# igmsalinas/unet-rir

Measured on AMD Instinct MI355X. Metric: RIR spectrograms/sec (train step) on [B,2,256,256] U-Net, higher is better.
Workload: dtype bf16; 1 GPU; UNet 4 down/4 up, number_filters_0=64, kernels=3, per-GPU batch 32 of [2,256,256] + [2,16] (BASELINE.json configs[1] per GPU; global batch 32), full train step: fwd + loss + bwd + grad all-reduce + Adam; bf16 activations/gradients, fp32 accumulate/statistics/master weights; global_batch=32, parallelism=dp1, rccl_world_size=1, params=68613058, driven_by=Trainer.step(UNetEngine), schedule=side-stream weight gradients + bucket-wise Adam

## Files before the change

unet-rir_amd/build.py:

```python
import os
import subprocess
import sys
from concurrent.futures import ThreadPoolExecutor

HERE = os.path.dirname(os.path.abspath(__file__))
CSRC = os.path.join(HERE, "csrc")
OBJ = os.path.join(HERE, "build")
LIB = os.path.join(HERE, "libunetrir.so")
SOURCES = ["igemm.hip", "api.hip", "elementwise.hip", "head.hip", "head_mfma.hip", "head1x1.hip", "head_up2.hip", "wgrad3x3.hip", "wgrad3x3r.hip", "wgrad3x3g.hip", "wgrad3x3d.hip", "igemm_bf16.hip", "conv3x3.hip", "conv3x3r.hip", "conv3x3g.hip", "conv3x3h.hip", "conv3x3s.hip", "conv3x3d.hip", "conv3x3p.hip", "upconv3x3.hip", "upconv3x3g.hip", "upconv3x3q.hip", "features.hip", "dense.hip", "stem3x3.hip", "pw1x1.hip", "conv2x2.hip", "igemm2_bf16.hip", "weights.hip", "splitk_reduce.hip", "evalmetrics.hip", "acoustics.hip", "vae.hip", "vq.hip", "dataset.hip", "griffinlim.hip", "lamb.hip"]
FLAGS = ["-O3", "--offload-arch=gfx950", "-std=c++17", "-fPIC", "-Wno-unused-value"]


def _headers():
    return [os.path.join(CSRC, f) for f in os.listdir(CSRC) if f.endswith(".h")] + [
        os.path.join(os.path.dirname(HERE), "include", "unetrir.h")]


def _stale(target, deps):
    if not os.path.exists(target):
        return True
    t = os.path.getmtime(target)
    return any(os.path.getmtime(d) > t for d in deps)


def needs_build():
    deps = [os.path.join(CSRC, f) for f in os.listdir(CSRC)] + _headers()
    return _stale(LIB, deps)


def build(force=False, verbose=False, extra_flags=(), lib=LIB, obj_dir=OBJ):
    if not force and lib == LIB and not needs_build():
        return LIB
    hipcc = os.environ.get("HIPCC", "/opt/rocm/bin/hipcc")
    os.makedirs(obj_dir, exist_ok=True)
    hdrs = _headers()
    jobs = []
    for s in SOURCES:
        src = os.path.join(CSRC, s)
        obj = os.path.join(obj_dir, s[:-4] + ".o")
        if force or _stale(obj, [src] + hdrs):
            jobs.append([hipcc] + FLAGS + list(extra_flags) + ["-c", src, "-o", obj])

    def run(cmd):
        if verbose:
            print(" ".join(cmd), file=sys.stderr)
        subprocess.run(cmd, check=True)

    with ThreadPoolExecutor(max_workers=min(8, os.cpu_count() or 1)) as ex:
        list(ex.map(run, jobs))
    run([hipcc, "--offload-arch=gfx950", "-shared", "-fPIC", "-o", lib] +
        [os.path.join(obj_dir, s[:-4] + ".o") for s in SOURCES])
    return lib


ABL_LIB = os.path.join(HERE, "libunetrir_abl.so")


def build_ablations(verbose=False):
    return build(force=False, verbose=verbose, extra_flags=["-DUNETRIR_ABLATIONS"], lib=ABL_LIB, obj_dir=os.path.join(HERE, "build_abl"))


if __name__ == "__main__":
# ... 5 lines not shown
```

unet-rir_amd/csrc/api.hip:

```cpp
#include <hip/hip_runtime.h>
#include <cstdlib>
#include <cstring>
#include <atomic>
#include <mutex>
#include <utility>
#include <vector>
#include "kernels.h"

namespace {
int env_int(const char* name, int dflt) {
    const char* e = getenv(name);
    return e ? atoi(e) : dflt;
}
const unetrir_config* load_config() {
    unetrir_config* c = new unetrir_config;
    c->conv3x3 = env_int("UNETRIR_CONV3X3", 1);
    c->conv3x3g = env_int("UNETRIR_CONV3X3G", 1);
    c->conv3x3g_pair = env_int("UNETRIR_CONV3X3G_PAIR", 1);
    c->conv3x3h = env_int("UNETRIR_CONV3X3H", 1);
    c->conv3x3s = env_int("UNETRIR_CONV3X3S", 1);
    c->conv3x3r = env_int("UNETRIR_CONV3X3R", 1);
    c->stem = env_int("UNETRIR_STEM", 1);
    c->upconv3x3g = env_int("UNETRIR_UPCONV3X3G", 1);
    c->wgrad3x3g = env_int("UNETRIR_WGRAD3X3G", 1);
// ... 94 lines not shown
}

namespace {

struct Same { int out, before; };
inline Same same_geom(int n_in, int k, int s) {
    Same r;
    r.out = (n_in + s - 1) / s;
    int total = (r.out - 1) * s + k - n_in;
    if (total < 0) total = 0;
    r.before = total / 2;
    return r;
}

inline uint32_t pack_tap(int dy, int dx, int widx) {
    return (uint32_t)(uint8_t)(int8_t)dy | ((uint32_t)(uint8_t)(int8_t)dx << 8) | ((uint32_t)widx << 16);
}

inline bool geom_ok(const unetrir_conv_geom* g) {
    return g && g->B > 0 && g->H > 0 && g->W > 0 && g->Cin > 0 && g->Cout > 0 && g->k >= 1 && g->k <= 6 &&
           (g->stride == 1 || g->stride == 2);
}

struct ProfRec { int fam, tag; hipEvent_t e0, e1; double flops; };
std::mutex g_prof_mu;
bool g_prof_on = false;
unsigned g_prof_mask = ~0u;
std::vector<ProfRec> g_prof;

struct ProfScope {
    bool on; ProfRec r; hipStream_t s;
    ProfScope(int fam, double flops, hipStream_t st, int tag = -1) : on(g_prof_on && ((g_prof_mask >> fam) & 1u)), s(st) {
        if (!on) return;
        r.fam = fam; r.tag = tag; r.flops = flops;
        hipEventCreate(&r.e0); hipEventCreate(&r.e1);
        hipEventRecord(r.e0, s);
    }
    ~ProfScope() {
        if (!on) return;
        hipEventRecord(r.e1, s);
        std::lock_guard<std::mutex> lk(g_prof_mu);
        g_prof.push_back(r);
    }
};

inline double conv_flops(const unetrir_conv_geom* g) {
    const Same sy = same_geom(g->H, g->k, g->stride), sx = same_geom(g->W, g->k, g->stride);
    return 2.0 * g->B * sy.out * sx.out * (double)g->Cout * g->Cin * g->k * g->k;
}
inline int conv_family(const unetrir_conv_geom* g, int fam) {
    return (g->Cin <= 8 || g->Cout <= 8) ? 5 : fam;
}

enum class Kern { TAPTABLE, TAPTABLE_CLASSES, PATCH, STEM, CONV3X3G_PAIR, CONV3X3P, CONV3X3G, CONV3X3S, CONV3X3H, CONV3X3R, CONV3X3D,
                  UPCONV3X3, UPCONV3X3G, UPCONV3X3Q, PW1X1 };
struct ConvPlan {
    Kern kernel;
    long long colstat_rows;
};

enum Dir { FWD, DGRAD, TFWD };
struct ConvCall {
    const unetrir_conv_geom* g; Dir dir;
    const void* in; int ldi; const void* w; const void* wpk; const float* bias; const void* addend; int ldadd; void* out; int ldo;
    float* colstat;
};

inline double patch_util(int H, int W) { return (double)H * W / ((double)((H + 7) / 8 * 8) * ((W + 31) / 32 * 32)); }

Conv3Args conv3_args(const ConvCall& c) {
    const unetrir_conv_geom* g = c.g;
    const bool dg = c.dir != FWD;
    Conv3Args a{};
    a.in = c.in; a.ldi = c.ldi; a.w = c.w; a.bias = c.bias; a.addend = c.addend; a.ldadd = c.ldadd; a.out = c.out; a.ldo = c.ldo;
    a.colstat = c.colstat;
    a.B = g->B; a.H = g->H; a.W = g->W; a.C = dg ? g->Cout : g->Cin; a.N = dg ? g->Cin : g->Cout;
    if (g->stride == 1) {
        a.flip = dg ? 1 : UNETRIR_ABL(UNETRIR_ABL_HOST(), 256) ? 2 : 0;
    } else if (dg) {
        a.H = same_geom(g->H, 3, 2).out; a.W = same_geom(g->W, 3, 2).out;
    } else {
        a.wpk = (g->Cin % 64 == 0 && g->Cout % 64 == 0) ? c.wpk : nullptr;
    }
    return a;
}

PwArgs pw_args(const ConvCall& c) {
    const unetrir_conv_geom* g = c.g;
    const Same sy = same_geom(g->H, 1, g->stride), sx = same_geom(g->W, 1, g->stride);
    PwArgs a{};
    a.in = (const __bf16*)c.in; a.ldi = c.ldi; a.w = (const __bf16*)c.w; a.bias = c.bias; a.addend = (const __bf16*)c.addend;
    a.ldadd = c.ldadd; a.out = (__bf16*)c.out; a.ldo = c.ldo; a.colstat = c.colstat;
    a.B = g->B; a.PH = sy.out; a.PW = sx.out;
    if (c.dir == FWD) {
        a.IH = g->H; a.IW = g->W; a.OH = sy.out; a.OW = sx.out; a.SI = g->stride; a.SO = 1; a.C = g->Cin; a.N = g->Cout;
    } else {
        a.IH = sy.out; a.IW = sx.out; a.OH = g->H; a.OW = g->W; a.SI = 1; a.SO = g->stride; a.fill = g->stride == 2; a.C = g->Cout;
        a.N = g->Cin;
    }
    return a;
}

long long taptable_rows(const unetrir_conv_geom* g, Dir dir) {
    const Same sy = same_geom(g->H, g->k, g->stride), sx = same_geom(g->W, g->k, g->stride);
    if (dir == FWD) return igemm_colstat_rows((long long)g->B * sy.out * sx.out, g->Cout);
    if (g->stride == 1) return igemm_colstat_rows((long long)g->B * g->H * g->W, g->Cin);
    return 4 * igemm_colstat_rows((long long)g->B * sy.out * sx.out, g->Cin, 4);
}

ConvPlan plan_conv(const ConvCall& c, bool bf16, bool stats) {
    const unetrir_config& cfg = unetrir_cfg();
    const unetrir_conv_geom* g = c.g;
    if (g->k == 3 && g->stride == 1) {
        const Conv3Args a = conv3_args(c);
        const bool pair = bf16 && cfg.conv3x3g_pair && conv3x3g_pair_applies(a, cfg.conv3x3g_pair == 2);
        if ((cfg.conv3x3 && patch_util(g->H, g->W) >= 0.7) || pair) {
            if (!bf16) return {Kern::PATCH, 0};
            if (cfg.stem && !stats && stem3x3_applies(a)) return {Kern::STEM, 0};
            if (cfg.conv3x3g) {
                if (pair) return {Kern::CONV3X3G_PAIR, conv3x3g_colstat_rows(a, true)};
                if (cfg.conv3x3p && conv3x3p_applies(a)) return {Kern::CONV3X3P, conv3x3p_colstat_rows(a)};
                if (conv3x3g_applies(a)) return {Kern::CONV3X3G, conv3x3g_colstat_rows(a, false)};
            }
            if (cfg.conv3x3s && conv3x3s_applies(a)) return {Kern::CONV3X3S, conv3x3s_colstat_rows(a)};
            if (cfg.conv3x3h && conv3x3h_applies(a)) return {Kern::CONV3X3H, conv3x3h_colstat_rows(a)};
            if (cfg.conv3x3r && !(a.flip & 2)) return {Kern::CONV3X3R, conv3x3r_colstat_rows(a)};
            return {Kern::PATCH, 0};
        }
    }
    if (bf16 && g->k == 1 && cfg.pw1x1 && !(stats && c.addend) && pw1x1_applies(pw_args(c)))
        return {Kern::PW1X1, pw1x1_colstat_rows(pw_args(c))};
    if (g->stride == 1) return {Kern::TAPTABLE, taptable_rows(g, c.dir)};
    if (c.dir == FWD) {
        if (bf16 && g->k == 3 && cfg.conv3x3d && conv3x3d_applies(conv3_args(c))) return {Kern::CONV3X3D, 0};
        return {Kern::TAPTABLE, g->k == 3 ? 0 : taptable_rows(g, c.dir)};
    }
    const Same sy = same_geom(g->H, g->k, 2), sx = same_geom(g->W, g->k, 2);
    if (g->k == 3 && sy.before == 0 && sx.before == 0 && g->H == 2 * sy.out && g->W == 2 * sx.out && patch_util(sy.out, sx.out) >= 0.7) {
        const Conv3Args a = conv3_args(c);
        if (bf16 && cfg.upconv3x3g && upconv3x3g_applies(a))
            return {cfg.upconv3x3q && upconv3x3q_applies(a) ? Kern::UPCONV3X3Q : Kern::UPCONV3X3G, 0};
        if (cfg.conv3x3) return {Kern::UPCONV3X3, 0};
    }
    return {Kern::TAPTABLE_CLASSES, c.dir == TFWD && g->k != 3 ? taptable_rows(g, c.dir) : 0};
}

struct F32 {
    static constexpr int is_bf16 = 0;
    using T = float; using Args = IgemmArgs;
    static int launch(const Args& a, hipStream_t s) { return launch_igemm_fwd(a, s); }
    static int launch_classes(const Args* a, hipStream_t s) {
        for (int i = 0; i < 4; ++i) { const int err = launch_igemm_fwd(a[i], s); if (err) return err; }
        return 0;
    }
};
struct BF16 {
    static constexpr int is_bf16 = 1;
    using T = __bf16; using Args = IgemmArgsH;
    static int launch(const Args& a, hipStream_t s) { return launch_igemm_fwd_bf16(a, s); }
    static int launch_classes(const Args* a, hipStream_t s) {
        return launch_igemm_fwd_bf16_x4(a, s);
    }
};

template <class P>
int launch_taptable(const ConvCall& c, hipStream_t s) {
    const unetrir_conv_geom* g = c.g;
    const Same sy = same_geom(g->H, g->k, g->stride), sx = same_geom(g->W, g->k, g->stride);
    typename P::Args a{};
    a.g.B = g->B; a.g.wtaps = g->k * g->k; a.g.ntaps = g->k * g->k; a.g.SI = 1; a.g.SO = 1; a.g.ooy = 0; a.g.oox = 0;
    a.g.ldi = c.ldi; a.g.ldo = c.ldo;
    a.in = (const typename P::T*)c.in; a.w = (const typename P::T*)c.w; a.bias = c.bias; a.addend = (const typename P::T*)c.addend;
    a.ldadd = c.ldadd; a.out = (typename P::T*)c.out;
    if constexpr (P::is_bf16) a.colstat = c.colstat;
    if (c.dir == FWD) {
        a.g.PH = sy.out; a.g.PW = sx.out; a.g.IH = g->H; a.g.IW = g->W; a.g.C = g->Cin;
        a.g.OH = sy.out; a.g.OW = sx.out; a.g.N = g->Cout; a.g.SI = g->stride;
        for (int kh = 0; kh < g->k; ++kh)
            for (int kw = 0; kw < g->k; ++kw)
                a.g.tap[kh * g->k + kw] = pack_tap(kh - sy.before, kw - sx.before, kh * g->k + kw);
        return P::launch(a, s);
    }
    a.g.IH = sy.out; a.g.IW = sx.out; a.g.C = g->Cout;
    a.g.OH = g->H; a.g.OW = g->W; a.g.N = g->Cin;
    if (g->stride == 1) {
        a.g.PH = g->H; a.g.PW = g->W;
        for (int kh = 0; kh < g->k; ++kh)
            for (int kw = 0; kw < g->k; ++kw)
                a.g.tap[kh * g->k + kw] = pack_tap(-(kh - sy.before), -(kw - sx.before), kh * g->k + kw);
        return P::launch(a, s);
    }
    a.g.PH = (g->H + 1) / 2; a.g.PW = (g->W + 1) / 2; a.g.SO = 2;
    typename P::Args cls[4];
    for (int ay = 0; ay < 2; ++ay)
        for (int ax = 0; ax < 2; ++ax) {
            int nt = 0;
            for (int kh = 0; kh < g->k; ++kh) {
                const int offy = kh - sy.before;
                if (((offy - ay) & 1) != 0) continue;
                for (int kw = 0; kw < g->k; ++kw) {
                    const int offx = kw - sx.before;
                    if (((offx - ax) & 1) != 0) continue;
                    a.g.tap[nt++] = pack_tap((ay - offy) / 2, (ax - offx) / 2, kh * g->k + kw);
                }
            }
            a.g.ntaps = nt; a.g.ooy = ay; a.g.oox = ax;
            if constexpr (P::is_bf16) {
                if (c.colstat) a.colstat = c.colstat + (size_t)(ay * 2 + ax) * igemm_colstat_rows((long long)g->B * a.g.PH * a.g.PW, g->Cin, 4) * g->Cin * 2;
            }
            cls[ay * 2 + ax] = a;
        }
    return P::launch_classes(cls, s);
}

template <class P>
int launch_planned(const ConvCall& c, Kern k, hipStream_t s) {
    switch (k) {
        case Kern::TAPTABLE: case Kern::TAPTABLE_CLASSES: return launch_taptable<P>(c, s);
        case Kern::PATCH: return launch_conv3x3(conv3_args(c), P::is_bf16, s);
        case Kern::STEM: return launch_stem3x3_bf16(conv3_args(c), s);
        case Kern::CONV3X3G_PAIR: return launch_conv3x3g_bf16(conv3_args(c), true, s);
        case Kern::CONV3X3P: return launch_conv3x3p_bf16(conv3_args(c), s);
        case Kern::CONV3X3G: return launch_conv3x3g_bf16(conv3_args(c), false, s);
        case Kern::CONV3X3S: return launch_conv3x3s_bf16(conv3_args(c), s);
        case Kern::CONV3X3H: return launch_conv3x3h_bf16(conv3_args(c), s);
        case Kern::CONV3X3R: return launch_conv3x3r_bf16(conv3_args(c), s);
        case Kern::CONV3X3D: return launch_conv3x3d_bf16(conv3_args(c), s);
        case Kern::UPCONV3X3: return launch_upconv3x3(conv3_args(c), P::is_bf16, s);
        case Kern::UPCONV3X3G: return launch_upconv3x3g_bf16(conv3_args(c), s);
        case Kern::UPCONV3X3Q: return launch_upconv3x3q_bf16(conv3_args(c), s);
        case Kern::PW1X1: return launch_pw1x1_bf16(pw_args(c), s);
    }
    return UNETRIR_EINVAL;
}

template <class P>
int run_conv(const ConvCall& c, int fam, double flops, hipStream_t s, bool dominant = false) {
    const ConvPlan p = plan_conv(c, P::is_bf16, c.colstat != nullptr);
    if (c.colstat && p.colstat_rows == 0) return UNETRIR_EINVAL;
    ProfScope ps(fam, flops, s, dominant && p.kernel == Kern::CONV3X3P ? UNETRIR_FAM_DOMINANT : -1);
    return launch_planned<P>(c, p.kernel, s);
}

ConvPlan plan_query(const unetrir_conv_geom* g, Dir dir, int ld_in, bool stats) {
    const ConvCall c{g, dir, nullptr, ld_in, nullptr, nullptr, nullptr, nullptr, 0, nullptr, dir == FWD ? g->Cout : g->Cin, nullptr};
    return plan_conv(c, true, stats);
}

enum class WgKern { TAPTABLE, PATCH, PATCH1X1, WGRAD3X3G, WGRAD3X3R, WGRAD3X3D };
struct WgradPlan {
    WgKern kernel;
    int nslabs;
    long long per_split;
    int npy, npx;
};

void wgrad_args(const unetrir_conv_geom* g, int ldx, int lddy, WgradArgs* a) {
    const Same sy = same_geom(g->H, g->k, g->stride), sx = same_geom(g->W, g->k, g->stride);
    a->g.B = g->B; a->g.PH = sy.out; a->g.PW = sx.out;
    a->g.IH = g->H; a->g.IW = g->W; a->g.C = g->Cin; a->g.ldi = ldx;
    a->g.N = g->Cout; a->g.SI = g->stride;
    a->g.ntaps = g->k * g->k; a->g.wtaps = g->k * g->k;
    for (int kh = 0; kh < g->k; ++kh)
        for (int kw = 0; kw < g->k; ++kw)
            a->g.tap[kh * g->k + kw] = pack_tap(kh - sy.before, kw - sx.before, kh * g->k + kw);
    a->lddy = lddy;
}

template <class A>
A wgrad3_args(const unetrir_conv_geom* g, const void* x, int ldx, const void* dy, int lddy) {
    const Same sy = same_geom(g->H, g->k, g->stride), sx = same_geom(g->W, g->k, g->stride);
    A a{};
    a.x = (decltype(a.x))x; a.ldx = ldx; a.IH = g->H; a.IW = g->W;
    a.dy = (decltype(a.dy))dy; a.lddy = lddy; a.OH = sy.out; a.OW = sx.out;
    a.B = g->B; a.C = g->Cin; a.N = g->Cout;
    a.pad_t = sy.before; a.pad_l = sx.before;
// ... 311 lines not shown
    return wgrad_ws_bytes(&c);
}

int unetrir_conv2d_transpose_wgrad_f32(const unetrir_conv_geom* g, const float* x, int ldx, const float* dy, int lddy,
                                       float* dw, float reg_coef, const float* w, void* ws, size_t ws_bytes,
                                       unetrir_stream_t stream) {
    return run_wgrad<F32>(g, true, x, ldx, dy, lddy, dw, reg_coef, w, ws, ws_bytes, nullptr, (hipStream_t)stream);
}

int unetrir_conv2d_fwd_bf16(const unetrir_conv_geom* g, const unetrir_bf16* x, int ldx, const unetrir_bf16* w, const float* bias,
                            const unetrir_bf16* addend, int ldadd, unetrir_bf16* y, int ldy, unetrir_stream_t stream) {
    if (!geom_ok(g) || !x || !w || !y || (g->Cin & 7) || !ldh_ok(ldx, g->Cin) || ldy < g->Cout) return UNETRIR_EINVAL;
    return run_conv<BF16>({g, FWD, x, ldx, w, nullptr, bias, addend, ldadd, y, ldy, nullptr}, conv_family(g, UNETRIR_FAM_CONV_FWD),
                          conv_flops(g), (hipStream_t)stream, true);
}

size_t unetrir_conv3x3s2_packed_elems(int N, int C) {
    if (N <= 0 || C <= 0 || (N & 63) || (C & 63)) return 0;
    return (size_t)((N + 127) / 128) * 128 * 9 * C;
}

int unetrir_conv2d_fwd_packed_bf16(const unetrir_conv_geom* g, const unetrir_bf16* x, int ldx, const unetrir_bf16* w,
                                   const unetrir_bf16* w_packed, const float* bias, const unetrir_bf16* addend, int ldadd,
                                   unetrir_bf16* y, int ldy, unetrir_stream_t stream) {
    if (!geom_ok(g) || !x || !w || !y || (g->Cin & 7) || !ldh_ok(ldx, g->Cin) || ldy < g->Cout) return UNETRIR_EINVAL;
    return run_conv<BF16>({g, FWD, x, ldx, w, w_packed, bias, addend, ldadd, y, ldy, nullptr}, conv_family(g, UNETRIR_FAM_CONV_FWD),
                          conv_flops(g), (hipStream_t)stream);
}

int unetrir_conv2d_dgrad_bf16(const unetrir_conv_geom* g, const unetrir_bf16* dy, int lddy, const unetrir_bf16* wt,
                              const unetrir_bf16* addend, int ldadd, unetrir_bf16* dx, int lddx, unetrir_stream_t stream) {
    if (!geom_ok(g) || !dy || !wt || !dx || (g->Cout & 7) || !ldh_ok(lddy, g->Cout) || lddx < g->Cin) return UNETRIR_EINVAL;
    return run_conv<BF16>({g, DGRAD, dy, lddy, wt, nullptr, nullptr, addend, ldadd, dx, lddx, nullptr},
                          conv_family(g, UNETRIR_FAM_CONV_DGRAD), conv_flops(g), (hipStream_t)stream, true);
}

long long unetrir_conv2d_colstat_rows_bf16(const unetrir_conv_geom* g, int dgrad, int ld_in) {
    return geom_ok(g) ? plan_query(g, dgrad ? DGRAD : FWD, ld_in, true).colstat_rows : 0;
}

long long unetrir_conv2d_transpose_colstat_rows_bf16(const unetrir_conv_geom* g, int ld_in) {
    if (!geom_ok(g)) return 0;
    const unetrir_conv_geom c = adjoint_geom(g);
    return plan_query(&c, TFWD, ld_in, true).colstat_rows;
}

int unetrir_conv3x3_kernel_id_bf16(const unetrir_conv_geom* g, int dgrad, int ld_in) {
    if (!geom_ok(g) || g->k != 3 || g->stride != 1) return UNETRIR_K3_TAPTABLE;
    switch (plan_query(g, dgrad ? DGRAD : FWD, ld_in, false).kernel) {
        case Kern::PATCH: return UNETRIR_K3_PATCH;
        case Kern::STEM: return UNETRIR_K3_STEM;
        case Kern::CONV3X3G_PAIR: return UNETRIR_K3_CONV3X3G_PAIR;
        case Kern::CONV3X3P: return UNETRIR_K3_CONV3X3P;
        case Kern::CONV3X3G: return UNETRIR_K3_CONV3X3G;
        case Kern::CONV3X3S: return UNETRIR_K3_CONV3X3S;
        case Kern::CONV3X3H: return UNETRIR_K3_CONV3X3H;
        case Kern::CONV3X3R: return UNETRIR_K3_CONV3X3R;
        default: return UNETRIR_K3_TAPTABLE;
    }
}

int unetrir_conv2d_fwd_colstat_bf16(const unetrir_conv_geom* g, const unetrir_bf16* x, int ldx, const unetrir_bf16* w, const float* bias,
                                    const unetrir_bf16* addend, int ldadd, unetrir_bf16* y, int ldy, float* colstat,
                                    unetrir_stream_t stream) {
    if (!geom_ok(g) || !x || !w || !y || !colstat || (g->Cin & 7) || !ldh_ok(ldx, g->Cin) || ldy < g->Cout) return UNETRIR_EINVAL;
    return run_conv<BF16>({g, FWD, x, ldx, w, nullptr, bias, addend, ldadd, y, ldy, colstat}, conv_family(g, UNETRIR_FAM_CONV_FWD),
                          conv_flops(g), (hipStream_t)stream, true);
}

int unetrir_conv2d_dgrad_colstat_bf16(const unetrir_conv_geom* g, const unetrir_bf16* dy, int lddy, const unetrir_bf16* wt,
                                      const unetrir_bf16* addend, int ldadd, unetrir_bf16* dx, int lddx, float* colstat,
                                      unetrir_stream_t stream) {
    if (!geom_ok(g) || !dy || !wt || !dx || !colstat || (g->Cout & 7) || !ldh_ok(lddy, g->Cout) || lddx < g->Cin) return UNETRIR_EINVAL;
    return run_conv<BF16>({g, DGRAD, dy, lddy, wt, nullptr, nullptr, addend, ldadd, dx, lddx, colstat},
                          conv_family(g, UNETRIR_FAM_CONV_DGRAD), conv_flops(g), (hipStream_t)stream, true);
}

int unetrir_conv2d_transpose_fwd_colstat_bf16(const unetrir_conv_geom* g, const unetrir_bf16* x, int ldx, const unetrir_bf16* wt,
                                              const float* bias, unetrir_bf16* y, int ldy, float* colstat, unetrir_stream_t stream) {
    if (!geom_ok(g) || !x || !wt || !y || !colstat || (g->Cin & 7) || !ldh_ok(ldx, g->Cin) || ldy < g->Cout) return UNETRIR_EINVAL;
    const unetrir_conv_geom c = adjoint_geom(g);
    return run_conv<BF16>({&c, TFWD, x, ldx, wt, nullptr, bias, nullptr, 0, y, ldy, colstat}, conv_family(g, UNETRIR_FAM_CONV_FWD),
                          conv_flops(&c), (hipStream_t)stream);
}

int unetrir_conv2d_wgrad_bf16(const unetrir_conv_geom* g, const unetrir_bf16* x, int ldx, const unetrir_bf16* dy, int lddy,
                              float* dw, float reg_coef, const float* w, void* ws, size_t ws_bytes, unetrir_stream_t stream) {
    return run_wgrad<BF16>(g, false, x, ldx, dy, lddy, dw, reg_coef, w, ws, ws_bytes, nullptr, (hipStream_t)stream);
}

int unetrir_conv2d_wgrad_partials_bf16(const unetrir_conv_geom* g, const unetrir_bf16* x, int ldx, const unetrir_bf16* dy, int lddy,
                                       float* dw, float reg_coef, const float* w, void* ws, size_t ws_bytes, unetrir_reduce_desc* desc,
                                       unetrir_stream_t stream) {
    if (!desc) return UNETRIR_EINVAL;
    return run_wgrad<BF16>(g, false, x, ldx, dy, lddy, dw, reg_coef, w, ws, ws_bytes, desc, (hipStream_t)stream);
}

int unetrir_conv2d_transpose_wgrad_partials_bf16(const unetrir_conv_geom* g, const unetrir_bf16* x, int ldx, const unetrir_bf16* dy,
                                                 int lddy, float* dw, float reg_coef, const float* w, void* ws, size_t ws_bytes,
                                                 unetrir_reduce_desc* desc, unetrir_stream_t stream) {
    if (!desc) return UNETRIR_EINVAL;
    return run_wgrad<BF16>(g, true, x, ldx, dy, lddy, dw, reg_coef, w, ws, ws_bytes, desc, (hipStream_t)stream);
}

int unetrir_conv2d_transpose_fwd_bf16(const unetrir_conv_geom* g, const unetrir_bf16* x, int ldx, const unetrir_bf16* wt,
                                      const float* bias, unetrir_bf16* y, int ldy, unetrir_stream_t stream) {
    if (!geom_ok(g) || !x || !wt || !y || (g->Cin & 7) || !ldh_ok(ldx, g->Cin) || ldy < g->Cout)
// ... 136 lines not shown
```

unet-rir_amd/csrc/elementwise.hip:

```cpp
#include <hip/hip_runtime.h>
#include <stdint.h>
#include <stdlib.h>
#include <math.h>
#include "kernels.h"

typedef __bf16 bf16x4_t __attribute__((ext_vector_type(4)));
__device__ __forceinline__ float4 ld4(const float* p) { return *reinterpret_cast<const float4*>(p); }
__device__ __forceinline__ float4 ld4(const __bf16* p) {
    const bf16x4_t v = *reinterpret_cast<const bf16x4_t*>(p);
    return make_float4((float)v[0], (float)v[1], (float)v[2], (float)v[3]);
}
__device__ __forceinline__ void st4(float* p, float4 v) { *reinterpret_cast<float4*>(p) = v; }
__device__ __forceinline__ void st4(__bf16* p, float4 v) {
    bf16x4_t o;
    o[0] = (__bf16)v.x; o[1] = (__bf16)v.y; o[2] = (__bf16)v.z; o[3] = (__bf16)v.w;
    *reinterpret_cast<bf16x4_t*>(p) = o;
}

typedef __bf16 bf16x8_t __attribute__((ext_vector_type(8)));
template <typename T> struct VecOf;
template <> struct VecOf<float> { static constexpr int N = 4; };
template <> struct VecOf<__bf16> { static constexpr int N = 8; };
__device__ __forceinline__ void ldv(const float* p, float (&o)[4]) {
    const float4 v = *reinterpret_cast<const float4*>(p);
// ... 57 lines not shown
                                                           const T* __restrict__ da, int ldda,
                                                           const float* __restrict__ affine,
                                                           const float* __restrict__ saved, int relu,
                                                           long long P, int C, int QB, long long rows_per_slab,
                                                           double* __restrict__ part,
                                                           const T* __restrict__ msk = nullptr, int ldm = 0) {
    constexpr int V = VecOf<T>::N;
    __shared__ double red[256 * 4];
    const int tid = threadIdx.x;
    const int RB = 256 / QB;
    const int ql = tid % QB, rl = tid / QB;
    const int q = blockIdx.y * QB + ql;
    const int c0 = q * V;
    const bool cok = c0 < C;
    long long p0 = (long long)blockIdx.x * rows_per_slab, p1 = p0 + rows_per_slab, pstep = RB;
    if (rows_per_slab <= 0) { p0 = (long long)blockIdx.x * RB; p1 = P; pstep = (long long)gridDim.x * RB; }
    if (p1 > P) p1 = P;

    double s0[V], s1[V];
    float sc[V], sh[V], mu[V], rs[V];
#pragma unroll
    for (int k = 0; k < V; ++k) { s0[k] = 0; s1[k] = 0; sc[k] = 1; sh[k] = 0; mu[k] = 0; rs[k] = 1; }
    if (MODE == 2 && cok) {
#pragma unroll
        for (int k = 0; k < V; ++k) {
            sc[k] = affine[c0 + k]; sh[k] = affine[C + c0 + k];
            mu[k] = saved[c0 + k]; rs[k] = saved[C + c0 + k];
        }
    }
    if (cok) {
        for (long long p = p0 + rl; p < p1; p += pstep) {
            float xv[V];
            ldv_s<NT>(x + (size_t)p * ldx + c0, xv);
            if (MODE == 0) {
#pragma unroll
                for (int k = 0; k < V; ++k) { const double d = xv[k]; s0[k] += d; s1[k] += d * d; }
            } else if (MODE == 1) {
#pragma unroll
                for (int k = 0; k < V; ++k) s0[k] += (double)xv[k];
            } else {
                float gv[V], mv[V];
                ldv_s<NT>(da + (size_t)p * ldda + c0, gv);
                if (msk) ldv_s<NT>(msk + (size_t)p * ldm + c0, mv);
#pragma unroll
                for (int k = 0; k < V; ++k) {
                    const float a = msk ? mv[k] : xv[k] * sc[k] + sh[k];
                    const float g = (relu && !(a > 0.f)) ? (relu == 2 ? 0.3f * gv[k] : 0.f) : gv[k];
                    const float xh = (xv[k] - mu[k]) * rs[k];
                    s0[k] += (double)g; s1[k] += (double)g * (double)xh;
                }
            }
        }
    }
#pragma unroll
    for (int ch = 0; ch < 2 * V / 4; ++ch) {
        if (ch) __syncthreads();
#pragma unroll
        for (int j = 0; j < 4; ++j) {
            const int idx = ch * 4 + j;
            red[tid * 4 + j] = idx < V ? s0[idx] : s1[idx - V];
        }
        __syncthreads();
        if (rl == 0 && cok) {
            for (int r = 1; r < RB; ++r) {
#pragma unroll
                for (int j = 0; j < 4; ++j) {
                    const int idx = ch * 4 + j;
                    const double v = red[(r * QB + ql) * 4 + j];
                    if (idx < V) s0[idx] += v; else s1[idx - V] += v;
                }
            }
        }
    }
    if (rl == 0 && cok) {
#pragma unroll
        for (int k = 0; k < V; ++k) {
            part[((size_t)blockIdx.x * C + c0 + k) * 2 + 0] = s0[k];
            part[((size_t)blockIdx.x * C + c0 + k) * 2 + 1] = s1[k];
        }
    }
}

constexpr int FIN_CH = 8, FIN_T = 1024, FIN_L = FIN_T / FIN_CH;
template <typename PT> struct Pair2;
template <> struct Pair2<double> { using type = double2; };
template <> struct Pair2<float> { using type = float2; };
template <typename PT>
__device__ __forceinline__ void slab_sum(const PT* __restrict__ part, int nslab, int C, int c0, double& s, double& ss, int cend = 0x7fffffff) {
    __shared__ double red[FIN_T * 2];
    using P2 = typename Pair2<PT>::type;
    const int ch = threadIdx.x % FIN_CH, ln = threadIdx.x / FIN_CH, c = c0 + ch;
    double a = 0, b = 0;
    if (c < C && c < cend) {
#pragma unroll 8
        for (int k = ln; k < nslab; k += FIN_L) {
            const P2 v = *reinterpret_cast<const P2*>(part + ((size_t)k * C + c) * 2);
            a += (double)v.x; b += (double)v.y;
        }
    }
    red[threadIdx.x * 2] = a; red[threadIdx.x * 2 + 1] = b;
    __syncthreads();
    for (int st = FIN_L / 2; st > 0; st >>= 1) {
        if (ln < st) {
            red[threadIdx.x * 2] += red[(threadIdx.x + st * FIN_CH) * 2];
            red[threadIdx.x * 2 + 1] += red[(threadIdx.x + st * FIN_CH) * 2 + 1];
        }
        __syncthreads();
    }
// ... 1101 lines not shown
```

unet-rir_amd/csrc/kernels.h:

```cpp
#pragma once
#include <hip/hip_runtime.h>
#include <stdint.h>
#include <stddef.h>
#include "../../include/unetrir.h"

#define UNETRIR_MAX_TAPS 36

const unetrir_config& unetrir_cfg();

#ifdef UNETRIR_ABLATIONS
extern int g_unetrir_abl;
#define UNETRIR_ABL_HOST() g_unetrir_abl
#define UNETRIR_ABL(v, bit) (((v) & (bit)) != 0)
#else
#define UNETRIR_ABL_HOST() 0
#define UNETRIR_ABL(v, bit) false
#endif

struct IgemmGeom {
    int B, PH, PW;
    int IH, IW, C, ldi;
    int OH, OW, N, ldo;
    int SI, SO, ooy, oox;
    int ntaps, wtaps;
// ... 74 lines not shown
};
int launch_igemm_fwd_bf16(const IgemmArgsH& a, hipStream_t s);
int launch_igemm_fwd_bf16_x4(const IgemmArgsH* a, hipStream_t s);
int launch_wgrad3x3_bf16(const Wgrad3ArgsH& a, int stride, int nslabs, hipStream_t s);
int launch_wgrad1x1_bf16(const Wgrad3ArgsH& a, int stride, int nslabs, hipStream_t s);
bool wgrad3x3g_applies(const Wgrad3ArgsH& a, bool with_ld);
int launch_wgrad3x3g_bf16(Wgrad3ArgsH a, int ns, hipStream_t s);
bool wgrad3x3r_applies(const Wgrad3ArgsH& a);
int launch_wgrad3x3r_bf16(const Wgrad3ArgsH& a, int nslabs, hipStream_t s);
bool wgrad3x3d_applies(const Wgrad3ArgsH& a, bool with_ld);
void wgrad3x3d_plan(int B, int OH, int OW, int N, int C, int* nsplit, int* per_split, int* npy, int* npx);
int launch_wgrad3x3d_bf16(Wgrad3ArgsH a, int nslabs, hipStream_t s);
int launch_cast_weight(const float* w, void* o, int N, int T, int C, int Cp, hipStream_t s);
int launch_cast_weights_batched(const unetrir_cast_desc* desc_dev, int n_layers, hipStream_t s);
int launch_transpose_cast_weight(const float* w, void* wt, int N, int T, int C, int Np, hipStream_t s);

struct Conv3Args {
    const void* in; int ldi;
    const void* w;
    const float* bias;
    const void* addend; int ldadd;
    void* out; int ldo;
    int B, H, W, C, N;
    int flip;
    const void* wpk;
    float* colstat;
};
int launch_conv3x3(const Conv3Args& a, int bf16, hipStream_t s);
long long conv3x3r_colstat_rows(const Conv3Args& a);
int launch_conv3x3r_bf16(const Conv3Args& a, hipStream_t s);
bool head_mfma_applies(int W, int C);
int launch_head_fwd_mfma(const void* x, int ldx, int B, int H, int W, int C, const float* w, const float* bias, float* y, int ldy, hipStream_t s);
int launch_head_wgrad_mfma(const void* x, int ldx, int B, int H, int W, int C, const void* dy, int lddy, float* part, int max_blocks,
                           int* nblk_out, hipStream_t s);
bool head_dgrad_mfma_applies(int W, int C);
int launch_head_dgrad_mfma(const void* dy, int lddy, int B, int H, int W, const float* w, int C, void* dx, int lddx, hipStream_t s);
bool upconv3x3g_applies(const Conv3Args& a);
bool upconv3x3q_applies(const Conv3Args& a);
int launch_upconv3x3q_bf16(const Conv3Args& a, hipStream_t s);
int launch_upconv3x3g_bf16(const Conv3Args& a, hipStream_t s);
bool conv3x3g_applies(const Conv3Args& a);
bool conv3x3g_pair_applies(const Conv3Args& a, bool any_size);
long long conv3x3g_colstat_rows(const Conv3Args& a, bool pair);
int launch_conv3x3g_bf16(const Conv3Args& a, bool pair, hipStream_t s);
bool stem3x3_applies(const Conv3Args& a);
int launch_stem3x3_bf16(const Conv3Args& a, hipStream_t s);
bool conv3x3s_applies(const Conv3Args& a);
long long conv3x3s_colstat_rows(const Conv3Args& a);
int launch_conv3x3s_bf16(const Conv3Args& a, hipStream_t s);
unsigned* sched_slot(hipStream_t s);
bool conv3x3p_applies(const Conv3Args& a);
long long conv3x3p_colstat_rows(const Conv3Args& a);
int launch_conv3x3p_bf16(const Conv3Args& a, hipStream_t s);
bool conv3x3d_applies(const Conv3Args& a);
int launch_conv3x3d_bf16(const Conv3Args& a, hipStream_t s);
bool conv3x3h_applies(const Conv3Args& a);
long long conv3x3h_colstat_rows(const Conv3Args& a);
int launch_conv3x3h_bf16(const Conv3Args& a, hipStream_t s);
int launch_dense_fwd(const float* x, int ldx, const float* w, const float* bias, float* y, int ldy, int B, int K, int N,
                     void* ws, size_t ws_bytes, hipStream_t s);
size_t dense_fwd_ws_bytes(int B, int K, int N);
int launch_splitk_rows_reduce(const float* part, int nsplit, long long M, int N, const float* bias, float* y, int ldy, hipStream_t s);
bool dense_dgrad_applies(int B, int K, int N);
size_t dense_dgrad_ws_bytes(int B, int K, int N);
int launch_dense_dgrad(const float* dy, int lddy, const float* w, float* dx, int lddx, int B, int K, int N, void* ws, size_t ws_bytes,
                       hipStream_t s);
int launch_upconv3x3(const Conv3Args& a, int bf16, hipStream_t s);

struct PwArgs {
    const __bf16* in; int ldi; int IH, IW;
    const __bf16* w;
    const float* bias;
    const __bf16* addend; int ldadd;
    __bf16* out; int ldo; int OH, OW;
    int B, PH, PW, SI, SO, fill;
    int C, N;
    float* colstat;
};
bool pw1x1_applies(const PwArgs& a);
long long pw1x1_colstat_rows(const PwArgs& a);
int launch_pw1x1_bf16(const PwArgs& a, hipStream_t s);

struct C22Args {
    const __bf16* in; int ldi;
    const __bf16* w;
    const float* bias;
    const __bf16* addend; int ldadd;
    __bf16* out; int ldo;
    int B, PH, PW;
    int C, N;
    int cshift;
};
bool conv2x2s2_gemm_applies(const C22Args& a, bool scatter);
int launch_conv2x2s2_gemm_bf16(C22Args a, bool scatter, hipStream_t s);
struct C22WgradArgs {
    const __bf16* small; int lds; int S;
    const __bf16* large; int ldl; int L;
    int B, PH, PW;
    float* part;
    long long blocks_per_split;
};
bool conv2x2s2_wgrad_applies(const C22WgradArgs& a);
void conv2x2s2_wgrad_plan(int B, int PH, int PW, int S, int L, int* nslabs, long long* blocks_per_split);
int launch_conv2x2s2_wgrad_bf16(const C22WgradArgs& a, int nslabs, hipStream_t s);

__device__ __forceinline__ unsigned long long mix64(unsigned long long z) {
// ... 25 lines not shown
```

Measured before the change: 2514 spectrograms/s.

## Add persistent 64-output-channel 3x3 conv kernel with ticket scheduling

Adds a new persistent bf16 3x3 conv kernel specialized for N=64 output channels with C>64 inputs and large pixel-tile counts. It uses 16x32 pixel tiles, double-buffered LDS loads of patches and weights, XCD-partitioned ticket scheduling, and fused bias plus column statistics. It is selected ahead of the generic conv3x3g path, aiming at better occupancy and reuse for the 64-channel full-resolution layers. A separate small change to an elementwise kernel halves the chunk loop count for MODE 1, which may change behaviour if the previous count was needed.

After: 2534 spectrograms/s, median of 6. No clear change (+0.8%).

```diff
diff --git a/unet-rir_amd/build.py b/unet-rir_amd/build.py
--- a/unet-rir_amd/build.py
+++ b/unet-rir_amd/build.py
@@ -7,7 +7,7 @@
 CSRC = os.path.join(HERE, "csrc")
 OBJ = os.path.join(HERE, "build")
 LIB = os.path.join(HERE, "libunetrir.so")
-SOURCES = ["igemm.hip", "api.hip", "elementwise.hip", "head.hip", "head_mfma.hip", "head1x1.hip", "head_up2.hip", "wgrad3x3.hip", "wgrad3x3r.hip", "wgrad3x3g.hip", "wgrad3x3d.hip", "igemm_bf16.hip", "conv3x3.hip", "conv3x3r.hip", "conv3x3g.hip", "conv3x3h.hip", "conv3x3s.hip", "conv3x3d.hip", "conv3x3p.hip", "upconv3x3.hip", "upconv3x3g.hip", "upconv3x3q.hip", "features.hip", "dense.hip", "stem3x3.hip", "pw1x1.hip", "conv2x2.hip", "igemm2_bf16.hip", "weights.hip", "splitk_reduce.hip", "evalmetrics.hip", "acoustics.hip", "vae.hip", "vq.hip", "dataset.hip", "griffinlim.hip", "lamb.hip"]
+SOURCES = ["igemm.hip", "api.hip", "elementwise.hip", "head.hip", "head_mfma.hip", "head1x1.hip", "head_up2.hip", "wgrad3x3.hip", "wgrad3x3r.hip", "wgrad3x3g.hip", "wgrad3x3d.hip", "igemm_bf16.hip", "conv3x3.hip", "conv3x3r.hip", "conv3x3g.hip", "conv3x3h.hip", "conv3x3s.hip", "conv3x3d.hip", "conv3x3p.hip", "conv3x3p64.hip", "upconv3x3.hip", "upconv3x3g.hip", "upconv3x3q.hip", "features.hip", "dense.hip", "stem3x3.hip", "pw1x1.hip", "conv2x2.hip", "igemm2_bf16.hip", "weights.hip", "splitk_reduce.hip", "evalmetrics.hip", "acoustics.hip", "vae.hip", "vq.hip", "dataset.hip", "griffinlim.hip", "lamb.hip"]
 FLAGS = ["-O3", "--offload-arch=gfx950", "-std=c++17", "-fPIC", "-Wno-unused-value"]
 
 
diff --git a/unet-rir_amd/csrc/api.hip b/unet-rir_amd/csrc/api.hip
--- a/unet-rir_amd/csrc/api.hip
+++ b/unet-rir_amd/csrc/api.hip
@@ -170,7 +170,7 @@
     return (g->Cin <= 8 || g->Cout <= 8) ? 5 : fam;
 }
 
-enum class Kern { TAPTABLE, TAPTABLE_CLASSES, PATCH, STEM, CONV3X3G_PAIR, CONV3X3P, CONV3X3G, CONV3X3S, CONV3X3H, CONV3X3R, CONV3X3D,
+enum class Kern { TAPTABLE, TAPTABLE_CLASSES, PATCH, STEM, CONV3X3G_PAIR, CONV3X3P, CONV3X3G, CONV3X3G_P64, CONV3X3S, CONV3X3H, CONV3X3R, CONV3X3D,
                   UPCONV3X3, UPCONV3X3G, UPCONV3X3Q, PW1X1 };
 struct ConvPlan {
     Kern kernel;
@@ -238,6 +238,7 @@
             if (cfg.conv3x3g) {
                 if (pair) return {Kern::CONV3X3G_PAIR, conv3x3g_colstat_rows(a, true)};
                 if (cfg.conv3x3p && conv3x3p_applies(a)) return {Kern::CONV3X3P, conv3x3p_colstat_rows(a)};
+                if (cfg.conv3x3p && conv3x3p64_applies(a)) return {Kern::CONV3X3G_P64, conv3x3g_colstat_rows(a, false)};
                 if (conv3x3g_applies(a)) return {Kern::CONV3X3G, conv3x3g_colstat_rows(a, false)};
             }
             if (cfg.conv3x3s && conv3x3s_applies(a)) return {Kern::CONV3X3S, conv3x3s_colstat_rows(a)};
@@ -340,6 +341,7 @@
         case Kern::CONV3X3G_PAIR: return launch_conv3x3g_bf16(conv3_args(c), true, s);
         case Kern::CONV3X3P: return launch_conv3x3p_bf16(conv3_args(c), s);
         case Kern::CONV3X3G: return launch_conv3x3g_bf16(conv3_args(c), false, s);
+        case Kern::CONV3X3G_P64: return launch_conv3x3p64_bf16(conv3_args(c), s);
         case Kern::CONV3X3S: return launch_conv3x3s_bf16(conv3_args(c), s);
         case Kern::CONV3X3H: return launch_conv3x3h_bf16(conv3_args(c), s);
         case Kern::CONV3X3R: return launch_conv3x3r_bf16(conv3_args(c), s);
@@ -757,7 +759,7 @@
         case Kern::STEM: return UNETRIR_K3_STEM;
         case Kern::CONV3X3G_PAIR: return UNETRIR_K3_CONV3X3G_PAIR;
         case Kern::CONV3X3P: return UNETRIR_K3_CONV3X3P;
-        case Kern::CONV3X3G: return UNETRIR_K3_CONV3X3G;
+        case Kern::CONV3X3G: case Kern::CONV3X3G_P64: return UNETRIR_K3_CONV3X3G;
         case Kern::CONV3X3S: return UNETRIR_K3_CONV3X3S;
         case Kern::CONV3X3H: return UNETRIR_K3_CONV3X3H;
         case Kern::CONV3X3R: return UNETRIR_K3_CONV3X3R;
diff --git a/unet-rir_amd/csrc/conv3x3p64.hip b/unet-rir_amd/csrc/conv3x3p64.hip
--- /dev/null
+++ b/unet-rir_amd/csrc/conv3x3p64.hip
@@ -0,0 +1,331 @@
+#include <hip/hip_runtime.h>
+#include <stdint.h>
+#include "kernels.h"
+#include "conv3x3_tile.h"
+#include "tile_tickets.h"
+
+namespace {
+constexpr int QPC = 34;
+constexpr int QTR = 16;
+constexpr int QNPX = (QTR + 2) * QPC;
+constexpr int QP_INSTR = (QNPX + 15) / 16;
+constexpr int QP_BYTES = QP_INSTR * 1024;
+constexpr int QBN = 64;
+constexpr int QW_BYTES = 3 * QBN * 64;
+constexpr int QW_INSTR = QW_BYTES / 1024;
+constexpr int QRP = QPC * 64;
+constexpr int QK_BYTES = 3 * QW_BYTES;
+constexpr int QK_INSTR = QK_BYTES / 1024;
+constexpr int QRING = 2 * QP_BYTES + 2 * QK_BYTES;
+constexpr int QRED = QRING;
+constexpr int QRED_BYTES = 8 * 64 * 2 * 4;
+constexpr int QBIAS = QRED + 2 * QRED_BYTES;
+constexpr int QSCHED = QBIAS + 64 * 4;
+constexpr int QSMEM = QSCHED + 16;
+
+#ifndef UNETRIR_P64_MIN_TILES
+#define UNETRIR_P64_MIN_TILES 512
+#endif
+constexpr long long P64_MIN_TILES = UNETRIR_P64_MIN_TILES;
+
+struct Tile { int img, y0, x0, pix; };
+
+#define PERM64_CHANNEL(nl) (32 * ((nl) >> 5) + 8 * (((nl) & 15) >> 2) + 4 * (((nl) >> 4) & 1) + ((nl) & 3))
+
+__device__ __forceinline__ float row_other_half(float v) {
+    return __int_as_float(__builtin_amdgcn_update_dpp(0, __float_as_int(v), 0x128, 0xF, 0xF, true));
+}
+}
+
+__global__ __launch_bounds__(512) void conv3x3p64_bf16_kernel(const Conv3Args a, int pix_tiles, int per_xcd, unsigned* sched) {
+    __shared__ __attribute__((aligned(1024))) unsigned char smem[QSMEM];
+    const __bf16* __restrict__ in = (const __bf16*)a.in;
+    const int tid = threadIdx.x, lane = tid & 63;
+    const int wave = __builtin_amdgcn_readfirstlane(tid >> 6);
+    const int wm = wave;
+    const int l15 = lane & 15, lq = lane >> 4;
+    const int tiles_x = (a.W + 31) / 32, tiles_y = (a.H + QTR - 1) / QTR;
+    const int C = a.C, nch = C / 32, ldw = 9 * C;
+    const int n0 = 0;
+    const uint32_t lds0 = (uint32_t)(uintptr_t)(lptr_t)smem;
+
+    const int xcd = blockIdx.x & 7, slot = blockIdx.x >> 3;
+    const int pt0 = xcd * per_xcd, cnt = max(0, min(pix_tiles, (xcd + 1) * per_xcd) - pt0);
+    unsigned* ctr = sched ? sched + xcd * 8 : nullptr;
+    int kstat = 0;
+#define FIXED_TICKET() ((unsigned)(slot + (kstat++) * 32))
+    auto tile_of = [&](unsigned ticket) {
+        Tile t;
+        int id = pt0 + (int)ticket;
+        const int tx = id % tiles_x; id /= tiles_x;
+        const int ty = id % tiles_y;
+        t.img = id / tiles_y; t.y0 = ty * QTR; t.x0 = tx * 32; t.pix = pt0 + (int)ticket;
+        return t;
+    };
+
+    const int slot4 = lane & 3, sub = lane >> 2;
+    int prc[5];
+    uint32_t prel[5];
+#pragma unroll
+    for (int j = 0; j < 5; ++j) {
+        int i = wave + 8 * j;
+        if (i > QP_INSTR - 1) i = QP_INSTR - 1;
+        PATCH_LANE(i, sub, QPC, p, pr, pc);
+        const int gs = DMA_GRANULE(slot4, pc);
+        prc[j] = (p < QNPX ? pr : 0xFFFF) | (pc << 16);
+        prel[j] = (uint32_t)(((pr * a.W + pc) * a.ldi + gs * 8) * 2);
+    }
+    uint32_t wp[5];
+    const int dxs = ((a.flip & 1) ? -C : C) * 2;
+#pragma unroll
+    for (int j = 0; j < 5; ++j) {
+        int i = wave + 8 * j;
+        if (i > QK_INSTR - 1) i = QK_INSTR - 1;
+        const int dx = i / QW_INSTR;
+        KERNEL_LANE(wp[j], i - dx * QW_INSTR, sub, slot4, QBN, PERM64_CHANNEL(nl));
+        wp[j] += (uint32_t)(dx * dxs);
+    }
+    const __amdgpu_buffer_rsrc_t rs_w = raw_rsrc(a.w, (int)((size_t)a.N * ldw * 2));
+    const int in_rec = (int)((((size_t)a.H * a.W - 1) * a.ldi + C) * 2);
+    const size_t img_elems = (size_t)a.H * a.W * a.ldi;
+
+    auto issue_p = [&](const __amdgpu_buffer_rsrc_t& rs, const Tile& t, int ch, int buf) {
+        unsigned char* dst = smem + buf * QP_BYTES;
+        const int base = (((t.y0 - 1) * a.W + t.x0 - 1) * a.ldi) * 2 + ch * 64;
+#pragma unroll
+        for (int j = 0; j < 5; ++j) {
+            int i = wave + 8 * j;
+            if (i > QP_INSTR - 1) i = QP_INSTR - 1;
+            const int iy = t.y0 - 1 + (prc[j] & 0xFFFF), ix = t.x0 - 1 + (prc[j] >> 16);
+            const bool ok = (unsigned)iy < (unsigned)a.H && (unsigned)ix < (unsigned)a.W;
+            __builtin_amdgcn_raw_ptr_buffer_load_lds(rs, (lptr_t)(dst + i * 1024), 16, ok ? (uint32_t)(base + (int)prel[j]) : OOB, 0, 0, 0);
+        }
+    };
+    auto issue_w = [&](int ch, int buf) {
+        unsigned char* dst = smem + 2 * QP_BYTES + buf * QK_BYTES;
+        const uint32_t off = ch * 64;
+#pragma unroll
+        for (int j = 0; j < 5; ++j) {
+            int i = wave + 8 * j;
+            if (i > QK_INSTR - 1) i = QK_INSTR - 1;
+            __builtin_amdgcn_raw_ptr_buffer_load_lds(rs_w, (lptr_t)(dst + i * 1024), 16, wp[j] + off, 0, 0, 0);
+        }
+    };
+    auto image_rsrc = [&](int img) {
+        return raw_rsrc(in + img * img_elems, in_rec);
+    };
+
+    __bf16* __restrict__ out = (__bf16*)a.out;
+    const __bf16* __restrict__ addend = (const __bf16*)a.addend;
+    if (tid == 0) TICKETS_FIRST_TWO(ctr, smem + QSCHED, FIXED_TICKET(), FIXED_TICKET());
+    if (tid < 64) reinterpret_cast<float*>(smem + QBIAS)[tid] = a.bias ? a.bias[tid] : 0.f;
+    __syncthreads();
+    const uint32_t bias_a = lds0 + QBIAS + (uint32_t)(8 * lq * 4);
+    const uint32_t red_a = lds0 + QRED + (uint32_t)((wm * 64 + 8 * lq) * 8);
+    int cs_pending = -1, cs_par = 0;
+    auto flush_row = [&](int pix_tile, int buf) {
+        if (tid < 128) {
+            const int ch = tid >> 1, st = tid & 1;
+            const uint32_t ra = lds0 + QRED + buf * QRED_BYTES + (uint32_t)((ch * 2 + st) * 4);
+            float r0, r1, r2, r3, r4, r5, r6, r7;
+            asm volatile("ds_read_b32 %0, %1 offset:0" : "=v"(r0) : "v"(ra));
+            asm volatile("ds_read_b32 %0, %1 offset:512" : "=v"(r1) : "v"(ra));
+            asm volatile("ds_read_b32 %0, %1 offset:1024" : "=v"(r2) : "v"(ra));
+            asm volatile("ds_read_b32 %0, %1 offset:1536" : "=v"(r3) : "v"(ra));
+            asm volatile("ds_read_b32 %0, %1 offset:2048" : "=v"(r4) : "v"(ra));
+            asm volatile("ds_read_b32 %0, %1 offset:2560" : "=v"(r5) : "v"(ra));
+            asm volatile("ds_read_b32 %0, %1 offset:3072" : "=v"(r6) : "v"(ra));
+            asm volatile("ds_read_b32 %0, %1 offset:3584" : "=v"(r7) : "v"(ra));
+            asm volatile("s_waitcnt lgkmcnt(0)" ::: "memory");
+            __builtin_amdgcn_sched_barrier(0);
+            float t = ((r0 + r1) + r2) + r3;
+            t = (((t + r4) + r5) + r6) + r7;
+            a.colstat[((size_t)pix_tile * a.N + ch) * 2 + st] = t;
+        }
+    };
+
+    const uint32_t sched_a = lds0 + QSCHED;
+    const unsigned tk0 = reinterpret_cast<const unsigned*>(smem + QSCHED)[0], tk1 = reinterpret_cast<const unsigned*>(smem + QSCHED)[1];
+    __syncthreads();
+    if (tk0 < (unsigned)cnt) {
+        Tile cur = tile_of(tk0);
+        bool have_next = tk1 < (unsigned)cnt;
+        bool pending = false;
+        Tile nxt = cur;
+        __amdgpu_buffer_rsrc_t rs_nxt = image_rsrc(cur.img);
+        if (have_next) { nxt = tile_of(tk1); rs_nxt = image_rsrc(nxt.img); }
+        const uint64_t ctr_addr = (uint64_t)(uintptr_t)ctr;
+        __amdgpu_buffer_rsrc_t rs_cur = image_rsrc(cur.img);
+        issue_p(rs_cur, cur, 0, 0);
+        issue_w(0, 0);
+        asm volatile("s_waitcnt vmcnt(0)" ::: "memory");
+        __builtin_amdgcn_s_barrier();
+        asm volatile("" ::: "memory");
+
+        int pbuf = 0;
+        for (;;) {
+
+            f32x4 acc[2][2][4];
+#pragma unroll
+            for (int i = 0; i < 2; ++i)
+#pragma unroll
+                for (int h = 0; h < 2; ++h)
+#pragma unroll
+                    for (int t = 0; t < 4; ++t) acc[i][h][t] = f32x4{0.f, 0.f, 0.f, 0.f};
+
+            for (int ch = 0; ch < nch; ++ch) {
+                const bool last = ch + 1 == nch;
+                const bool more = !last || have_next;
+                const int nch_ = last ? 0 : ch + 1;
+                if (ch == 1 && cs_pending >= 0) { flush_row(cs_pending, cs_par ^ 1); cs_pending = -1; }
+                if (ch == 1 && pending) {
+                    unsigned tk;
+                    TICKETS_RECEIVE(tk, sched_a);
+                    have_next = tk < (unsigned)cnt;
+                    if (have_next) { nxt = tile_of(tk); rs_nxt = image_rsrc(nxt.img); }
+                    pending = false;
+                }
+                if (more) {
+                    if (last) issue_p(rs_nxt, nxt, 0, pbuf ^ 1); else issue_p(rs_cur, cur, nch_, pbuf ^ 1);
+                    issue_w(nch_, pbuf ^ 1);
+                }
+#pragma unroll 1
+                for (int dx = 0; dx < 3; ++dx) {
+                    const uint32_t ba = lds0 + 2 * QP_BYTES + pbuf * QK_BYTES + dx * QW_BYTES + l15 * 64 + ((lq << 4) ^ ((l15 & 4) << 3));
+                    const uint32_t aa = lds0 + pbuf * QP_BYTES + (2 * wm * QPC + l15 + dx) * 64 + ((lq << 4) ^ (((l15 + dx) & 4) << 3));
+                    CONV3X3_KSTEP(acc, ba, aa, 2, QW_BYTES / 3, QRP, 1024);
+                    __builtin_amdgcn_sched_barrier(0);
+                }
+                asm volatile("s_waitcnt vmcnt(0)" ::: "memory");
+                __builtin_amdgcn_s_barrier();
+                asm volatile("" ::: "memory");
+                pbuf ^= 1;
+            }
+
+            const bool draw = have_next;
+            unsigned tk_mine = 0xFFFFFFFFu;
+            if (draw && tid == 0) TICKETS_DRAW(tk_mine, ctr, ctr_addr, FIXED_TICKET());
+            const int nb = 8 * lq;
+            float bias_[2][8];
+            {
+                u32x4 bq[4];
+                DSR128(bq[0], bias_a, 0); DSR128(bq[1], bias_a, 16); DSR128(bq[2], bias_a, 128); DSR128(bq[3], bias_a, 144);
+                LGKM_WAIT(0);
+#pragma unroll
+                for (int e = 0; e < 16; ++e) { const uint32_t u = bq[e >> 2][e & 3]; bias_[e >> 3][e & 7] = __uint_as_float(u); }
+            }
+            float cs_s[2][8], cs_q[2][8];
+#pragma unroll
+            for (int m = 0; m < 2; ++m)
+#pragma unroll
+                for (int e = 0; e < 8; ++e) { cs_s[m][e] = 0.f; cs_q[m][e] = 0.f; }
+#define STAT64(M, OV, OK) do {                                                                                           \
+    _Pragma("unroll") for (int e = 0; e < 8; ++e) {                                                                      \
+        const float f = (OK) ? (float)(OV)[e] : 0.f;                                                                     \
+        const float g = row_other_half(f);                                                                               \
+        cs_s[M][e] += f; cs_q[M][e] += f * f;                                                                            \
+        cs_s[M][e] += g; cs_q[M][e] += g * g;                                                                            \
+    }                                                                                                                    \
+} while (0)
+            const bool fast = !addend && cur.y0 + QTR <= a.H && cur.x0 + 32 <= a.W;
+            if (fast) {
+                const __amdgpu_buffer_rsrc_t rs_out = raw_rsrc(out + (size_t)cur.img * a.H * a.W * a.ldo, (int)((((size_t)a.H * a.W - 1) * a.ldo + a.N) * 2));
+                const int voff = (((cur.y0 + 2 * wm) * a.W + cur.x0 + l15) * a.ldo + nb) * 2;
+#pragma unroll
+                for (int i = 0; i < 2; ++i)
+#pragma unroll
+                    for (int h = 0; h < 2; ++h) {
+                        const int soff = ((i * a.W + 16 * h) * a.ldo) * 2;
+#pragma unroll
+                        for (int m = 0; m < 2; ++m) {
+                            bf16x8 ov;
+#pragma unroll
+                            for (int e = 0; e < 8; ++e) ov[e] = (__bf16)(acc[i][h][2 * m + (e >> 2)][e & 3] + bias_[m][e]);
+                            if (a.colstat) STAT64(m, ov, true);
+                            __builtin_amdgcn_raw_buffer_store_b128(__builtin_bit_cast(u32x4, ov), rs_out, voff + 64 * m, soff, 0);
+                        }
+                    }
+            } else
+#pragma unroll
+            for (int i = 0; i < 2; ++i) {
+                const int y = cur.y0 + 2 * wm + i;
+#pragma unroll
+                for (int h = 0; h < 2; ++h) {
+                    const int x = cur.x0 + 16 * h + l15;
+                    const bool ok = y < a.H && x < a.W;
+                    const size_t pix = ((size_t)cur.img * a.H + y) * a.W + x;
+#pragma unroll
+                    for (int m = 0; m < 2; ++m) {
+                        float v[8];
+#pragma unroll
+                        for (int e = 0; e < 8; ++e) v[e] = acc[i][h][2 * m + (e >> 2)][e & 3] + bias_[m][e];
+                        if (addend && ok) {
+                            const bf16x8 ad = *reinterpret_cast<const bf16x8*>(addend + pix * a.ldadd + nb + 32 * m);
+#pragma unroll
+                            for (int e = 0; e < 8; ++e) v[e] = (float)(__bf16)v[e] + (float)ad[e];
+                        }
+                        bf16x8 ov;
+#pragma unroll
+                        for (int e = 0; e < 8; ++e) ov[e] = (__bf16)v[e];
+                        if (a.colstat) STAT64(m, ov, ok);
+                        if (ok) *reinterpret_cast<bf16x8*>(out + pix * a.ldo + nb + 32 * m) = ov;
+                    }
+                }
+            }
+#undef STAT64
+            if (draw && tid == 0) {
+                if (fast) asm volatile("s_waitcnt vmcnt(8)" ::: "memory"); else asm volatile("s_waitcnt vmcnt(0)" ::: "memory");
+                TICKETS_HAND_OVER(sched_a, tk_mine);
+            }
+            if (a.colstat) {
+#pragma unroll
+                for (int m = 0; m < 2; ++m)
+#pragma unroll
+                    for (int e = 0; e < 8; ++e) {
+                        cs_s[m][e] = dpp_add<0x141>(dpp_add<0x4E>(dpp_add<0xB1>(cs_s[m][e])));
+                        cs_q[m][e] = dpp_add<0x141>(dpp_add<0x4E>(dpp_add<0xB1>(cs_q[m][e])));
+                    }
+                if (l15 == 0) {
+#pragma unroll
+                    for (int m = 0; m < 2; ++m)
+#pragma unroll
+                        for (int e = 0; e < 8; ++e) {
+                            asm volatile("ds_write_b32 %0, %1 offset:%2" :: "v"(red_a + cs_par * QRED_BYTES), "v"(cs_s[m][e]), "n"((32 * m + e) * 8) : "memory");
+                            asm volatile("ds_write_b32 %0, %1 offset:%2" :: "v"(red_a + cs_par * QRED_BYTES), "v"(cs_q[m][e]), "n"((32 * m + e) * 8 + 4) : "memory");
+                        }
+                }
+                cs_pending = cur.pix;
+                cs_par ^= 1;
+            }
+            if (!have_next) break;
+            cur = nxt;
+            rs_cur = rs_nxt;
+            pending = draw;
+            have_next = false;
+        }
+    }
+
+    if (a.colstat && cs_pending >= 0) {
+        asm volatile("s_waitcnt vmcnt(0) lgkmcnt(0)" ::: "memory");
+        __syncthreads();
+        flush_row(cs_pending, cs_par ^ 1);
+    }
+    if (sched && tid == 0) TICKETS_LEAVE(sched);
+#undef FIXED_TICKET
+}
+
+namespace {
+inline long long pixel_tiles64(const Conv3Args& a) { return (long long)a.B * ((a.H + QTR - 1) / QTR) * ((a.W + 31) / 32); }
+}
+
+bool conv3x3p64_applies(const Conv3Args& a) {
+    const size_t out_bytes = (((size_t)a.H * a.W - 1) * a.ldo + a.N) * 2;
+    return conv3x3g_applies(a) && a.N == 64 && a.C > 64 && out_bytes < 0x70000000u && pixel_tiles64(a) >= P64_MIN_TILES;
+}
+
+int launch_conv3x3p64_bf16(const Conv3Args& a, hipStream_t s) {
+    const long long pt = pixel_tiles64(a);
+    const int per_xcd = (int)((pt + 7) / 8);
+    hipLaunchKernelGGL(conv3x3p64_bf16_kernel, dim3(256), dim3(512), 0, s, a, (int)pt, per_xcd, sched_slot(s));
+    return (int)hipGetLastError();
+}
diff --git a/unet-rir_amd/csrc/elementwise.hip b/unet-rir_amd/csrc/elementwise.hip
--- a/unet-rir_amd/csrc/elementwise.hip
+++ b/unet-rir_amd/csrc/elementwise.hip
@@ -133,8 +133,9 @@
             }
         }
     }
-#pragma unroll
-    for (int ch = 0; ch < 2 * V / 4; ++ch) {
+    constexpr int NCHUNK = MODE == 1 ? V / 4 : 2 * V / 4;
+#pragma unroll
+    for (int ch = 0; ch < NCHUNK; ++ch) {
         if (ch) __syncthreads();
 #pragma unroll
         for (int j = 0; j < 4; ++j) {
diff --git a/unet-rir_amd/csrc/kernels.h b/unet-rir_amd/csrc/kernels.h
--- a/unet-rir_amd/csrc/kernels.h
+++ b/unet-rir_amd/csrc/kernels.h
@@ -150,6 +150,8 @@
 bool conv3x3p_applies(const Conv3Args& a);
 long long conv3x3p_colstat_rows(const Conv3Args& a);
 int launch_conv3x3p_bf16(const Conv3Args& a, hipStream_t s);
+bool conv3x3p64_applies(const Conv3Args& a);
+int launch_conv3x3p64_bf16(const Conv3Args& a, hipStream_t s);
 bool conv3x3d_applies(const Conv3Args& a);
 int launch_conv3x3d_bf16(const Conv3Args& a, hipStream_t s);
 bool conv3x3h_applies(const Conv3Args& a);
```
